# frankenz/Deep-convolutional-neural-network-ResNet-26-and-Attention-network

Measured on AMD Instinct MI355X. Metric: tiles/sec fwd+bwd, 256x256x3 bags, ResNet-26+attn, higher is better.
Workload: dtype bf16; 1 GPU; 8 bags x 256 tiles @256x256x3 per GPU, ResNet-26 (20/40/60/80) + attention-MIL head, fwd+bwd full-bag path (BASELINE.json configs[1]); global_bags=8, tiles_per_bag=256, tile=256, parallelism=bag-parallel dp1, one RCCL all-reduce of the flat 2.56 MB gradient bucket

## Files before the change

deep-convolutional-neural-network-resnet-26-and-attention-network_amd/csrc/conv_resident.hip:

```cpp
#include "pf_common.cuh"
#include <cstdlib>

struct ResConv {
    const __bf16* w;
    const float* bias;
    const __bf16* res;
    const __bf16* act;
    __bf16* out;
    int lrelu;
};
#define MIL_CHAIN_MAX 6
struct ResArgs {
    const __bf16* x;
    ResConv conv[MIL_CHAIN_MAX];
    int nconv;
    int n_img, ngroups;
    unsigned bytes;
    float slope;
};

constexpr int MIL_RES_BDEPTH = 2;

template <int C, int S, int IMGS>
struct ResGeom {
    static constexpr int CG = C / 8, NT = C / 16;
    static constexpr int PIX = mil_pix_pitch(C, 2);
    static constexpr int HS = S + 2;
    static constexpr int IMG = HS * HS * PIX;
    static constexpr int TILE = IMGS * IMG;
    static constexpr int KSTEPS = (9 * CG + 3) / 4;
    static constexpr int NPIX = IMGS * S * S;
    static constexpr int TILES = (NPIX + 15) / 16;
    static constexpr int MW = ((TILES + 7) / 8 + 1) / 2 * 2;
    static constexpr bool RAGGED = (S * S) % 16 != 0 || TILES != 8 * MW;
    static constexpr int NPIECE = NPIX * CG;
    static constexpr int NP = (NPIECE + 511) / 512;
    static constexpr bool WAVE_IS_IMAGE = !RAGGED && (S * S / 16 == MW);
    static_assert(C % 16 == 0, "shape");
    static_assert(TILE <= 160 * 1024, "LDS");
};

template <int C, int S, int IMGS>
__global__ __launch_bounds__(512, 2) void conv_resident_kernel(ResArgs a) {
    using G = ResGeom<C, S, IMGS>;
    constexpr int CG = G::CG, NT = G::NT, PIX = G::PIX, HS = G::HS, IMG = G::IMG, KSTEPS = G::KSTEPS, MW = G::MW, NP = G::NP, NPIX = G::NPIX;
    extern __shared__ __attribute__((aligned(16))) char tile[];
    MIL_POISON(tile);
    const int tid = threadIdx.x, lane = tid & 63;
    const int wave = __builtin_amdgcn_readfirstlane(tid >> 6);
    const int r = lane & 15, gq = lane >> 4;
    const __amdgpu_buffer_rsrc_t rs_x = mil_rsrc(a.x, a.bytes);

    unsigned sink = 0;
    for (int k = 0; k < a.nconv; ++k) {
        const __amdgpu_buffer_rsrc_t rs_wk = mil_rsrc(a.conv[k].w, KSTEPS * NT * 1024);
        for (int line = tid; line < KSTEPS * NT * 8; line += 512)
            sink ^= __builtin_amdgcn_raw_buffer_load_b32(rs_wk, (unsigned)line * 128u, 0, 0);
    }
    {
        constexpr int NB = 4 * S + 4, PPR = PIX / 16;
        for (int idx = tid; idx < IMGS * NB * PPR; idx += 512) {
            const int bp = idx / PPR, j = idx - bp * PPR;
            const int im = bp / NB, b = bp - im * NB;
            int hy, hx;
            if (b < HS) { hy = 0; hx = b; }
            else if (b < 2 * HS) { hy = HS - 1; hx = b - HS; }
            else { hy = 1 + ((b - 2 * HS) >> 1); hx = ((b - 2 * HS) & 1) * (HS - 1); }
            *reinterpret_cast<u32x4_t*>(tile + im * IMG + (hy * HS + hx) * PIX + j * 16) = u32x4_t{0u, 0u, 0u, 0u};
        }
    }
    int pixbase[MW];
#pragma unroll
    for (int m = 0; m < MW; ++m) {
        int P = (wave * MW + m) * 16 + r;
        if (G::RAGGED && P >= NPIX) P = NPIX - 1;
        const int im = P / (S * S), p = P - im * (S * S);
        pixbase[m] = im * IMG + ((p / S) * HS + (p % S)) * PIX;
    }
    const int c_off = (gq >> 1) * 16;

    for (int grp = blockIdx.x; grp < a.ngroups; grp += gridDim.x) {
        const int img0 = grp * IMGS;
        if (grp != (int)blockIdx.x) __syncthreads();
        {
            u32x4_t v[NP];
            const unsigned g0 = (unsigned)img0 * (unsigned)(S * S * C * 2);
#pragma unroll
            for (int i = 0; i < NP; ++i) v[i] = __builtin_amdgcn_raw_buffer_load_b128(rs_x, g0 + (unsigned)(tid + 512 * i) * 16u, 0, 0);
#pragma unroll
            for (int i = 0; i < NP; ++i) {
                const int idx = tid + 512 * i, pl = idx / CG, j = idx - pl * CG;
                const int im = pl / (S * S), p = pl - im * (S * S);
                if (!G::RAGGED || idx < G::NPIECE)
                    *reinterpret_cast<u32x4_t*>(tile + im * IMG + (((p / S) + 1) * HS + (p % S) + 1) * PIX + j * 16) = v[i];
            }
        }

        auto run_conv = [&](const ResConv& cv, bool to_lds, bool first) {
            const __amdgpu_buffer_rsrc_t rs_w = mil_rsrc(cv.w, KSTEPS * NT * 1024);
            const __amdgpu_buffer_rsrc_t rs_res = mil_rsrc(cv.res, cv.res ? a.bytes : 0);
            const __amdgpu_buffer_rsrc_t rs_act = mil_rsrc(cv.act, cv.act ? a.bytes : 0);
            const __amdgpu_buffer_rsrc_t rs_out = mil_rsrc(cv.out, a.bytes);
            f32x4_t acc[MW][NT];
#pragma unroll
            for (int nt = 0; nt < NT; ++nt) {
                f32x4_t b;
#pragma unroll
                for (int i = 0; i < 4; ++i) b[i] = cv.bias ? cv.bias[nt * 16 + gq * 4 + i] : 0.f;
#pragma unroll
                for (int m = 0; m < MW; ++m) acc[m][nt] = b;
            }
            constexpr int BD = MIL_RES_BDEPTH;
            Frag8<BF16> bq[BD + 1][NT], aq[2][MW];
            auto fetch_b = [&](int ks) {
#pragma unroll
                for (int nt = 0; nt < NT; ++nt)
                    bq[ks % (BD + 1)][nt].v = __builtin_bit_cast(bf16x8_t, __builtin_amdgcn_raw_buffer_load_b128(rs_w, (unsigned)(lane * 16), (ks * NT + nt) * 1024, 0));
            };
            auto off_ks = [&](int ks) {
                const int q = 4 * ks + gq;
                const int tap = q / CG, cg = q - tap * CG;
                const int ty = (tap * 11) >> 5, tx = tap - ty * 3;
                return q < 9 * CG ? (ty * HS + tx) * PIX + cg * 16 : 0;
            };
            auto fetch_a = [&](int ks) {
                const int off = off_ks(ks);
#pragma unroll
                for (int m = 0; m < MW; ++m) aq[ks & 1][m] = lds_frag<BF16>(tile + pixbase[m] + off);
            };
#pragma unroll
            for (int ks = 0; ks < BD; ++ks) fetch_b(ks);
            if (first || !G::WAVE_IS_IMAGE) __syncthreads();
            fetch_a(0);
#pragma unroll
            for (int ks = 0; ks < KSTEPS; ++ks) {
                if (ks + BD < KSTEPS) fetch_b(ks + BD);
                if (ks + 1 < KSTEPS) fetch_a(ks + 1);
                __builtin_amdgcn_sched_barrier(0);
#pragma unroll
                for (int m = 0; m < MW; ++m)
#pragma unroll
                    for (int nt = 0; nt < NT; ++nt) acc[m][nt] = mma8(bq[ks % (BD + 1)][nt], aq[ks & 1][m], acc[m][nt]);
                __builtin_amdgcn_sched_barrier(0);
            }
            if (to_lds && !G::WAVE_IS_IMAGE) __syncthreads();
#pragma unroll
            for (int p = 0; p < MW / 2; ++p) {
                const int P = (wave * MW + 2 * p + (gq & 1)) * 16 + r;
                const bool in_list = !G::RAGGED || P < NPIX;
                const int Pc = in_list ? P : NPIX - 1, im = Pc / (S * S), px = Pc - im * (S * S);
                const bool img_ok = in_list && img0 + im < a.n_img;
                const unsigned goff = img_ok ? (unsigned)(((img0 + im) * (S * S) + px) * (C * 2) + c_off) : MIL_OOB;
                u32x4_t rr[NT], ra[NT];
#pragma unroll
                for (int nt = 0; nt < NT; ++nt) {
                    if (cv.res) rr[nt] = __builtin_amdgcn_raw_buffer_load_b128(rs_res, goff == MIL_OOB ? MIL_OOB : goff + nt * 32, 0, 0);
                    if (cv.act) ra[nt] = __builtin_amdgcn_raw_buffer_load_b128(rs_act, goff == MIL_OOB ? MIL_OOB : goff + nt * 32, 0, 0);
                }
                const int loff = im * IMG + (((px / S) + 1) * HS + (px % S) + 1) * PIX + c_off;
#pragma unroll
                for (int nt = 0; nt < NT; ++nt) {
                    float v[8];
#pragma unroll
                    for (int i = 0; i < 4; ++i) {
                        float lo = acc[2 * p][nt][i], hi = acc[2 * p + 1][nt][i];
                        if (i == 0) mil_swap16<true>(lo, hi); else mil_swap16<false>(lo, hi);
                        v[i] = lo;
                        v[4 + i] = hi;
                    }
                    if (cv.res) {
                        const bf16x8_t tt = __builtin_bit_cast(bf16x8_t, rr[nt]);
#pragma unroll
                        for (int i = 0; i < 8; ++i) v[i] += (float)tt[i];
                    }
                    if (cv.lrelu) {
#pragma unroll
                        for (int i = 0; i < 8; ++i) v[i] = fmaxf(v[i], v[i] * a.slope);
                    }
                    if (cv.act) {
                        const bf16x8_t tt = __builtin_bit_cast(bf16x8_t, ra[nt]);
#pragma unroll
                        for (int i = 0; i < 8; ++i) v[i] *= ((float)tt[i] > 0.f ? 1.f : a.slope);
                    }
                    bf16x8_t ov;
#pragma unroll
                    for (int i = 0; i < 8; ++i) ov[i] = (__bf16)v[i];
                    const u32x4_t ou = __builtin_bit_cast(u32x4_t, ov);
                    __builtin_amdgcn_raw_buffer_store_b128(ou, rs_out, goff == MIL_OOB ? MIL_OOB : goff + nt * 32, 0, 0);
                    if (to_lds && in_list) *reinterpret_cast<u32x4_t*>(tile + loff + nt * 32) = img_ok ? ou : u32x4_t{0u, 0u, 0u, 0u};
                }
            }
        };
#pragma unroll 1
        for (int k = 0; k < a.nconv; ++k) run_conv(a.conv[k], k + 1 < a.nconv, k == 0);
    }
    asm volatile("" :: "v"(sink));
}

static int mil_res_grid_cap(int grid) {
    const char* e = mil_test_knob("MIL_RES_GRID_CAP");
    const int cap = e ? atoi(e) : 0;
    return (cap > 0 && grid > cap) ? cap : grid;
}

#include "conv_resident_x3.cuh"

template <int C, int S, int IMGS>
static int launch_resident(ResArgs a, hipStream_t st) {
    using G = ResGeom<C, S, IMGS>;
    auto kern = conv_resident_kernel<C, S, IMGS>;
    if (hipFuncSetAttribute(reinterpret_cast<const void*>(kern), hipFuncAttributeMaxDynamicSharedMemorySize, G::TILE) != hipSuccess)
        return MIL_ERR_LAUNCH;
    a.ngroups = (a.n_img + IMGS - 1) / IMGS;
    int grid = mil_num_cus();
    if (grid > a.ngroups) grid = a.ngroups;
    grid = mil_res_grid_cap(grid);
    hipLaunchKernelGGL(kern, dim3(grid), dim3(512), G::TILE, st, a);
    MIL_CHECK_LAUNCH();
    return MIL_OK;
}

static int resident_dispatch(ResArgs a, int cp, int H, int W, hipStream_t st) {
    if ((size_t)a.n_img * H * W * cp * 2 >= ((size_t)1 << 31)) return MIL_ERR_UNSUPPORTED;
    a.bytes = (unsigned)((size_t)a.n_img * H * W * cp * 2);
    if (cp == 80 && H == 8 && W == 8) return launch_resident<80, 8, 8>(a, st);
    if (cp == 64 && H == 16 && W == 16) return launch_resident<64, 16, 3>(a, st);
    if (cp == 80 && H == 10 && W == 10) return launch_resident<80, 10, 5>(a, st);
    if (cp == 64 && H == 19 && W == 19) return launch_resident<64, 19, 2>(a, st);
    return MIL_ERR_UNSUPPORTED;
}

int mil_resident_conv(const void* x, const void* wpack, const float* bias_pad, const void* res, const void* act, void* y, int n_img,
                      int H, int W, int cp, int apply_lrelu, float slope, hipStream_t st) {
    if (n_img <= 0 || slope < 0.f || slope >= 1.f) return MIL_ERR_UNSUPPORTED;
    if (cp != 80) return MIL_ERR_UNSUPPORTED;
    ResArgs a{};
    a.x = (const __bf16*)x; a.n_img = n_img; a.slope = slope; a.nconv = 1;
    a.conv[0].w = (const __bf16*)wpack; a.conv[0].bias = bias_pad; a.conv[0].res = (const __bf16*)res; a.conv[0].act = (const __bf16*)act;
    a.conv[0].out = (__bf16*)y; a.conv[0].lrelu = apply_lrelu;
    return resident_dispatch(a, cp, H, W, st);
}

int mil_resident_conv_x3(const void* x, const void* wpack, const float* bias_pad, const void* res, const void* act, void* y, int n_img,
                         int H, int W, int cp, int apply_lrelu, float slope, hipStream_t st) {
    if (n_img <= 0 || slope < 0.f || slope >= 1.f) return MIL_ERR_UNSUPPORTED;
    ResArgsX3 a{};
    a.x = (const float*)x; a.n_img = n_img; a.slope = slope; a.nconv = 1;
    a.conv[0].w = (const char*)wpack; a.conv[0].bias = bias_pad; a.conv[0].res = (const float*)res; a.conv[0].act = (const float*)act;
    a.conv[0].out = (float*)y; a.conv[0].lrelu = apply_lrelu;
    return resident_dispatch_x3(a, cp, H, W, st);
}

struct MilChainConv {
    const void* wpack; const float* bias; const void* res; const void* act; void* out; int lrelu; int pad_;
};
extern "C" int mil_conv_chain(const void* x, const MilChainConv* convs, int nconv, int n_img, int H, int W, int cp, float slope,
                              int dtype, void* stream) {
    if (!x || !convs || nconv < 1 || nconv > MIL_CHAIN_MAX || n_img < 0) return MIL_ERR_ARG;
    for (int k = 0; k < nconv; ++k) if (!convs[k].wpack || !convs[k].out) return MIL_ERR_ARG;
    if ((dtype != MIL_DT_BF16 && dtype != MIL_DT_F32S) || slope < 0.f || slope >= 1.f) return MIL_ERR_UNSUPPORTED;
    if (n_img == 0) return MIL_OK;
    if (dtype == MIL_DT_F32S) {
        ResArgsX3 b{};
        b.x = (const float*)x; b.n_img = n_img; b.slope = slope; b.nconv = nconv;
        for (int k = 0; k < nconv; ++k) {
            b.conv[k].w = (const char*)convs[k].wpack; b.conv[k].bias = convs[k].bias; b.conv[k].res = (const float*)convs[k].res;
            b.conv[k].act = (const float*)convs[k].act; b.conv[k].out = (float*)convs[k].out; b.conv[k].lrelu = convs[k].lrelu;
        }
        return resident_dispatch_x3(b, cp, H, W, reinterpret_cast<hipStream_t>(stream));
    }
    ResArgs a{};
    a.x = (const __bf16*)x; a.n_img = n_img; a.slope = slope; a.nconv = nconv;
    for (int k = 0; k < nconv; ++k) {
        a.conv[k].w = (const __bf16*)convs[k].wpack; a.conv[k].bias = convs[k].bias; a.conv[k].res = (const __bf16*)convs[k].res;
        a.conv[k].act = (const __bf16*)convs[k].act; a.conv[k].out = (__bf16*)convs[k].out; a.conv[k].lrelu = convs[k].lrelu;
    }
    return resident_dispatch(a, cp, H, W, reinterpret_cast<hipStream_t>(stream));
}

extern "C" int mil_conv_pair(const void* x, const void* wpackA, const float* biasA, const void* resA, const void* actA,
                             int lreluA, void* outA, const void* wpackB, const float* biasB, const void* resB,
                             const void* actB, int lreluB, void* outB, int n_img, int H, int W, int cp, float slope,
                             int dtype, void* stream) {
    if (!x || !wpackA || !wpackB || !outA || !outB || n_img < 0) return MIL_ERR_ARG;
    const MilChainConv c[2] = {{wpackA, biasA, resA, actA, outA, lreluA, 0}, {wpackB, biasB, resB, actB, outB, lreluB, 0}};
    return mil_conv_chain(x, c, 2, n_img, H, W, cp, slope, dtype, stream);
}
```

deep-convolutional-neural-network-resnet-26-and-attention-network_amd/ops.py:

```python
import ctypes

import torch

from . import _lib as L

LEAK = 0.1


class KernelTimer:

    def __init__(self, want):
        self.want = want
        self.spans = []

    def bracket(self, label):
        if not self.want(label):
            return None
        start = torch.cuda.Event(enable_timing=True)
        end = torch.cuda.Event(enable_timing=True)
        start.record()
        self.spans.append((label, start, end))
        return end

    def durations_ms(self):
        torch.cuda.synchronize()
        return [(label, s.elapsed_time(e)) for label, s, e in self.spans]


TIMER = None


class ReduceBatch:
    MAX_JOBS = 64

    def __init__(self, device):
        self.device = device
        self.rec = L.lib().mil_reduce_job_bytes()
        self.host = (ctypes.c_char * (self.rec * self.MAX_JOBS))()
        self.dev = torch.empty(self.rec * self.MAX_JOBS, dtype=torch.uint8, device=device)
        self.uploaded = None
        self.ws = {}
        self.handed = None

    def workspace(self, key, nbytes):
        if self.handed is not None:
            if key in self.handed:
                raise RuntimeError(f"slab workspace {key!r} handed out twice inside one deferred-reduction block: the second "
                                   "producer would overwrite slabs the batched reduction has not read yet")
            self.handed.add(key)
        t = self.ws.get(key)
        if t is None or t.numel() * 4 < nbytes:
            t = self.ws[key] = torch.empty((nbytes + 3) // 4, dtype=torch.float32, device=self.device)
        return t

    def __enter__(self):
        L.check(L.lib().mil_reduce_defer_begin(ctypes.addressof(self.host), self.MAX_JOBS), "mil_reduce_defer_begin")
        self.handed = set()
        return self

    def __exit__(self, exc_type, exc, tb):
        n = ctypes.c_int(0)
        self.handed = None
        L.check(L.lib().mil_reduce_defer_end(ctypes.byref(n)), "mil_reduce_defer_end")
        if exc_type is not None or n.value == 0:
            return False
        raw = bytes(self.host[: self.rec * n.value])
        if raw != self.uploaded:
            self.dev[: len(raw)].copy_(torch.frombuffer(bytearray(raw), dtype=torch.uint8))
            self.uploaded = raw
        L.check(L.lib().mil_wgrad_reduce_all(self.dev.data_ptr(), ctypes.addressof(self.host), n.value, L.stream_ptr()),
                "mil_wgrad_reduce_all")
        return False


def cpad(c):
    return (c + 7) // 8 * 8


def _need(t, shape, dtype, name):
    if t is None:
        return
    if not t.is_cuda or not t.is_contiguous():
        raise ValueError(f"{name} must be a contiguous CUDA tensor")
    if tuple(t.shape) != tuple(shape) or t.dtype != dtype:
        raise ValueError(f"{name}: expected {tuple(shape)} {dtype}, got {tuple(t.shape)} {t.dtype}")


def stem_s2d(x, dtype):
    if x.dim() != 4 or x.shape[1] != 3 or x.dtype != torch.float32 or not x.is_cuda:
        raise ValueError(f"expected a CUDA fp32 [N,3,H,W] tile stack, got {tuple(x.shape)} {x.dtype} on {x.device}")
    x = x.contiguous()
    n, _, h, w = x.shape
    out = torch.empty((n, (h + 1) // 2, (w + 1) // 2, 16), dtype=dtype, device=x.device)
    L.check(L.lib().mil_stem_s2d(x.data_ptr(), out.data_ptr(), n, h, w, L.dt_code(dtype), L.stream_ptr()), "mil_stem_s2d")
    return out


def _need_u8_tiles(x):
    if x.dim() != 4 or x.shape[1] != 3 or x.dtype != torch.uint8 or not x.is_cuda or not x.is_contiguous():
        raise ValueError(f"expected a contiguous CUDA uint8 [N,3,H,W] tile stack, got {tuple(x.shape)} {x.dtype} on {x.device}")


def stem_s2d_u8(x, dtype):
    _need_u8_tiles(x)
    n, _, h, w = x.shape
    out = torch.empty((n, (h + 1) // 2, (w + 1) // 2, 16), dtype=dtype, device=x.device)
    L.check(L.lib().mil_stem_s2d_u8(x.data_ptr(), out.data_ptr(), n, h, w, L.dt_code(dtype), L.stream_ptr()), "mil_stem_s2d_u8")
    return out


def pack_weights(w, bias, mode, dtype):
    w = w.detach()
    if w.dtype != torch.float32 or not w.is_cuda or w.dim() != 4:
        raise ValueError("weights must be CUDA fp32 [Cout,Cin,k,k]")
    w = w.contiguous()
    cout, cin, ks, _ = w.shape
    elems = ctypes.c_size_t(0)
    L.check(L.lib().mil_packed_weight_elems(ctypes.byref(elems), cout, cin, ks, mode), "mil_packed_weight_elems")
    if dtype == L.BF16X3:
        with L.f32_mma(L.MIL_DT_F32S):
            return pack_weights(w, bias, mode, torch.float32)
    packed = torch.empty(elems.value, dtype=dtype, device=w.device)
    n_out = cin if mode == L.PACK_DGRAD else cout
    nt = (cpad(n_out) + 15) // 16
    bias_pad = torch.empty(nt * 16, dtype=torch.float32, device=w.device)
    b = None if bias is None else bias.detach().contiguous()
    L.check(L.lib().mil_pack_conv_weights(w.data_ptr(), L.ptr(b), packed.data_ptr(), bias_pad.data_ptr(), cout, cin, ks,
                                          mode, L.dt_code(dtype, mma=True), L.stream_ptr()), "mil_pack_conv_weights")
    return packed, bias_pad


def conv(x, wpack, bias_pad, cout_p, *, ks, stride, pad, out_hw=None, res=None, act=None, lrelu=False,
         zero_insert=False, slope=LEAK):
    n, h, w, cin_p = x.shape
    if zero_insert:
        if out_hw is None:
            raise ValueError("zero_insert needs the full-resolution output size")
        ho, wo = out_hw
    else:
        ho = (h + 2 * pad - ks) // stride + 1 if ks != 4 else h
        wo = (w + 2 * pad - ks) // stride + 1 if ks != 4 else w
    y = torch.empty((n, ho, wo, cout_p), dtype=x.dtype, device=x.device)
    _need(x, x.shape, x.dtype, "x")
    _need(res, y.shape, x.dtype, "res")
    _need(act, y.shape, x.dtype, "act")
    end = TIMER.bracket(("conv", cin_p, cout_p, ks, stride, bool(zero_insert), n, ho, wo)) if TIMER else None
    L.check(L.lib().mil_conv_igemm(x.data_ptr(), wpack.data_ptr(), L.ptr(bias_pad), L.ptr(res), L.ptr(act), y.data_ptr(),
                                   n, h, w, cin_p, ho, wo, cout_p, ks, 1 if zero_insert else stride, pad,
                                   1 if zero_insert else 0, 1 if lrelu else 0, slope, L.dt_code(x.dtype, mma=True), L.stream_ptr()),
            "mil_conv_igemm")
    if end is not None:
        end.record()
    return y


def wgrad_workspace_bytes(n, h, w, cin, ho, wo, cout, ks, stride, pad, stem, dtype):
    need = ctypes.c_size_t(0)
    L.check(L.lib().mil_conv_wgrad_workspace(ctypes.byref(need), n, h, w, cin, ho, wo, cout, ks, stride, pad,
                                             1 if stem else 0, L.dt_code(dtype, mma=True)), "mil_conv_wgrad_workspace")
    return need.value


def conv_wgrad(x, dz, cin, cout, *, ks, stride, pad, stem=False, want_bias=True, workspace=None, out=None):
    n, h, w, cin_p = x.shape
    _, ho, wo, cout_p = dz.shape
    _need(dz, (n, ho, wo, cpad(cout)), x.dtype, "dz")
    _need(x, (n, h, w, 16 if stem else cpad(cin)), x.dtype, "x")
    need = wgrad_workspace_bytes(n, h, w, cin, ho, wo, cout, ks, stride, pad, stem, x.dtype)
    if workspace is None or workspace.numel() * workspace.element_size() < need:
        workspace = torch.empty((need + 3) // 4, dtype=torch.float32, device=x.device)
    kk = 7 if stem else ks
    if out is None:
        dw = torch.empty((cout, cin, kk, kk), dtype=torch.float32, device=x.device)
        db = torch.empty(cout, dtype=torch.float32, device=x.device) if want_bias else None
    else:
        dw, db = out
        _need(dw, (cout, cin, kk, kk), torch.float32, "dw")
        _need(db, (cout,), torch.float32, "db")
    end = TIMER.bracket(("wgrad", cin_p, cout_p, ks, stride, n, ho, wo)) if TIMER else None
    L.check(L.lib().mil_conv_wgrad(x.data_ptr(), dz.data_ptr(), dw.data_ptr(), L.ptr(db), workspace.data_ptr(),
                                   workspace.numel() * workspace.element_size(), n, h, w, cin, ho, wo, cout, ks, stride,
                                   pad, 1 if stem else 0, 0 if out is None else 1, L.dt_code(x.dtype, mma=True), L.stream_ptr()),
            "mil_conv_wgrad")
    if end is not None:
        end.record()
    return dw, db


def bwd_fused_workspace_bytes(n, h, w, cout, cin, ks, pad, dtype, dense=False):
    need = ctypes.c_size_t(0)
    rc = L.lib().mil_conv_bwd_fused_workspace(ctypes.byref(need), n, h, w, cout, cin, ks, pad, L.dt_code(dtype, dense, mma=True))
    if rc == 2:
        return None
    L.check(rc, "mil_conv_bwd_fused_workspace")
    return need.value


def conv_bwd_fused(dz, wpack_dgrad, x, cin, cout, *, addend=None, mask=True, ks=3, pad=1, workspace=None, slope=LEAK,
                   out=None):
    n, h, w, cz = dz.shape
    dense = cz == cout and cpad(cout) != cout
    need = bwd_fused_workspace_bytes(n, h, w, cout, cin, ks, pad, dz.dtype, dense)
    if need is None:
        return None
    _need(dz, (n, h, w, cout if dense else cpad(cout)), dz.dtype, "dz")
    _need(x, (n, h, w, cpad(cin)), dz.dtype, "x")
    _need(addend, (n, h, w, cin if dense else cpad(cin)), dz.dtype, "addend")
    if workspace is None or workspace.numel() * workspace.element_size() < need:
        workspace = torch.empty((need + 3) // 4, dtype=torch.float32, device=dz.device)
    dx = torch.empty((n, h, w, cin), dtype=dz.dtype, device=dz.device) if dense else torch.empty_like(x)
    if out is None:
        dw = torch.empty((cout, cin, ks, ks), dtype=torch.float32, device=dz.device)
        db = torch.empty(cout, dtype=torch.float32, device=dz.device)
    else:
        dw, db = out
        _need(dw, (cout, cin, ks, ks), torch.float32, "dw")
        _need(db, (cout,), torch.float32, "db")
    end = TIMER.bracket(("bwd_fused", cpad(cout), cpad(cin), ks, 1, False, n, h, w, addend is not None)) if TIMER else None
    L.check(L.lib().mil_conv_bwd_fused(dz.data_ptr(), wpack_dgrad.data_ptr(), x.data_ptr(), L.ptr(addend), dx.data_ptr(),
                                       dw.data_ptr(), db.data_ptr(), workspace.data_ptr(),
                                       workspace.numel() * workspace.element_size(), n, h, w, cout, cin, ks, pad,
                                       1 if mask else 0, 0 if out is None else 1, slope, L.dt_code(dz.dtype, dense, mma=True), L.stream_ptr()),
            "mil_conv_bwd_fused")
    if end is not None:
        end.record()
    return dx, dw, db


def maxpool_fwd(x):
    n, h, w, cp = x.shape
    ho, wo = (h - 1) // 2 + 1, (w - 1) // 2 + 1
    y = torch.empty((n, ho, wo, cp), dtype=x.dtype, device=x.device)
    widx = torch.empty((n, ho, wo, cp), dtype=torch.uint8, device=x.device)
    L.check(L.lib().mil_maxpool_fwd(x.data_ptr(), y.data_ptr(), widx.data_ptr(), n, h, w, cp, L.dt_code(x.dtype),
                                    L.stream_ptr()), "mil_maxpool_fwd")
    return y, widx


def maxpool_bwd(gy, widx, in_hw, lrelu_mask=True, slope=LEAK):
    n, ho, wo, cp = widx.shape
    h, w = in_hw
    if ((h - 1) // 2 + 1, (w - 1) // 2 + 1) != (ho, wo):
        raise ValueError(f"pool input {h}x{w} does not produce {ho}x{wo}")
    _need(gy, widx.shape, gy.dtype, "gy")
    gx = torch.empty((n, h, w, cp), dtype=gy.dtype, device=gy.device)
    L.check(L.lib().mil_maxpool_bwd(gy.data_ptr(), widx.data_ptr(), gx.data_ptr(), n, h, w, cp, 1 if lrelu_mask else 0,
                                    slope, L.dt_code(gy.dtype), L.stream_ptr()), "mil_maxpool_bwd")
    return gx


BLOCK_FWD_CHANNELS = (24,)


def conv_block_fwd(x, wpack1, bias1, wpack2, bias2, *, slope=LEAK):
    n, h, w, cp = x.shape
    code = L.dt_code(x.dtype, mma=True)
    if code == L.MIL_DT_F32S:
        if cp != 24 or h < 8 or w < 16:
            return None
    elif x.dtype != torch.bfloat16 or cp not in BLOCK_FWD_CHANNELS or h < 16 or w < 16:
        return None
    _need(x, x.shape, x.dtype, "x")
    o1 = torch.empty_like(x)
    y = torch.empty_like(x)
    end = TIMER.bracket(("block_fwd", cp, n, h, w)) if TIMER else None
    rc = L.lib().mil_conv_block_fwd(x.data_ptr(), wpack1.data_ptr(), L.ptr(bias1), wpack2.data_ptr(), L.ptr(bias2),
                                    o1.data_ptr(), y.data_ptr(), n, h, w, cp, slope, code, L.stream_ptr())
    if rc == 2:
        return None
    L.check(rc, "mil_conv_block_fwd")
    if end is not None:
        end.record()
    return o1, y


RESIDENT_SHAPES = ((80, 8, 8), (64, 16, 16), (80, 10, 10), (64, 19, 19))


class _ChainConv(ctypes.Structure):
    _fields_ = [("wpack", ctypes.c_void_p), ("bias", ctypes.c_void_p), ("res", ctypes.c_void_p), ("act", ctypes.c_void_p),
                ("out", ctypes.c_void_p), ("lrelu", ctypes.c_int), ("pad_", ctypes.c_int)]


def conv_chain(x, convs, *, slope=LEAK):
    n, h, w, cp = x.shape
    code = L.dt_code(x.dtype, mma=True)
    if code not in (L.MIL_DT_BF16, L.MIL_DT_F32S) or (cp, h, w) not in RESIDENT_SHAPES or not 1 <= len(convs) <= 6:
        return None
    _need(x, x.shape, x.dtype, "x")
    outs = [torch.empty_like(x) for _ in convs]
    arr = (_ChainConv * len(convs))()
    for k, c in enumerate(convs):
        ops_ = {}
        for name in ("res", "act"):
            t = c.get(name)
            if isinstance(t, int):
                if not 0 <= t < k:
                    raise ValueError(f"conv {k}: {name} refers to conv {t}, which is not earlier in the chain")
                t = outs[t]
            _need(t, x.shape, x.dtype, name)
            ops_[name] = t
        arr[k].wpack = c["w"].data_ptr()
        arr[k].bias = L.ptr(c.get("bias"))
        arr[k].res, arr[k].act = L.ptr(ops_["res"]), L.ptr(ops_["act"])
        arr[k].out = outs[k].data_ptr()
        arr[k].lrelu = 1 if c.get("lrelu") else 0
    end = TIMER.bracket(("chain", cp, n, h, w, len(convs))) if TIMER else None
    rc = L.lib().mil_conv_chain(x.data_ptr(), ctypes.addressof(arr), len(convs), n, h, w, cp, slope, code, L.stream_ptr())
    if rc == 2:
        return None
    L.check(rc, "mil_conv_chain")
    if end is not None:
        end.record()
    return outs


def conv_pair(x, wA, biasA, wB, biasB, *, resA=None, actA=None, lreluA=False, resB=None, actB=None, lreluB=False, slope=LEAK):
    outs = conv_chain(x, [dict(w=wA, bias=biasA, res=resA, act=actA, lrelu=lreluA),
                          dict(w=wB, bias=biasB, res=resB, act=actB, lrelu=lreluB)], slope=slope)
    return None if outs is None else (outs[0], outs[1])


def conv_s2_entry(x, wpack3, bias_pad, wpack1, cout_p, *, slope=LEAK):
    n, h, w, cin_p = x.shape
    code = L.dt_code(x.dtype, mma=True)
    if code not in (L.MIL_DT_BF16, L.MIL_DT_F32S):
        return None
    _need(x, x.shape, x.dtype, "x")
    ho, wo = (h - 1) // 2 + 1, (w - 1) // 2 + 1
    y1 = torch.empty((n, ho, wo, cout_p), dtype=x.dtype, device=x.device)
    y2 = torch.empty_like(y1)
    end = TIMER.bracket(("s2_entry", cin_p, cout_p, n, h, w)) if TIMER else None
    rc = L.lib().mil_conv_s2_entry(x.data_ptr(), wpack3.data_ptr(), L.ptr(bias_pad), wpack1.data_ptr(), y1.data_ptr(),
                                   y2.data_ptr(), n, h, w, cin_p, cout_p, slope, code, L.stream_ptr())
    if rc == 2:
        return None
    L.check(rc, "mil_conv_s2_entry")
    if end is not None:
        end.record()
    return y1, y2


def conv_wgrad_pair(x, dz1, dz2, cin, cout, *, workspace=None, out=None):
    n, h, w, _ = x.shape
    _, ho, wo, _ = dz1.shape
    code = L.dt_code(x.dtype, mma=True)
    if code not in (L.MIL_DT_BF16, L.MIL_DT_F32S):
        return None
    _need(x, (n, h, w, cpad(cin)), x.dtype, "x")
    _need(dz1, (n, ho, wo, cpad(cout)), x.dtype, "dz1")
    _need(dz2, (n, ho, wo, cpad(cout)), x.dtype, "dz2")
    need = ctypes.c_size_t(0)
    rc = L.lib().mil_conv_wgrad_pair_workspace(ctypes.byref(need), n, h, w, cin, ho, wo, cout, code)
    if rc == 2:
        return None
    L.check(rc, "mil_conv_wgrad_pair_workspace")
    if workspace is None or workspace.numel() * workspace.element_size() < need.value:
        workspace = torch.empty((need.value + 3) // 4, dtype=torch.float32, device=x.device)
    if out is None:
        dw3 = torch.empty((cout, cin, 3, 3), dtype=torch.float32, device=x.device)
        db3 = torch.empty(cout, dtype=torch.float32, device=x.device)
        dw1 = torch.empty((cout, cin, 1, 1), dtype=torch.float32, device=x.device)
    else:
        dw3, db3, dw1 = out
        _need(dw3, (cout, cin, 3, 3), torch.float32, "dw3")
        _need(db3, (cout,), torch.float32, "db3")
        _need(dw1, (cout, cin, 1, 1), torch.float32, "dw1")
    rc = L.lib().mil_conv_wgrad_pair(x.data_ptr(), dz1.data_ptr(), dz2.data_ptr(), dw3.data_ptr(), db3.data_ptr(), dw1.data_ptr(),
                                     workspace.data_ptr(), workspace.numel() * workspace.element_size(), n, h, w, cin, ho, wo,
                                     cout, 0 if out is None else 1, code, L.stream_ptr())
    if rc == 2:
        return None
    L.check(rc, "mil_conv_wgrad_pair")
    return dw3, db3, dw1, workspace


def conv_dgrad_s2(dz1, dz2, wpack, cx_p, out_hw, *, act=None, slope=LEAK, dense_cx=None):
    n, h, w, cz_p = dz1.shape
    hh, ww = out_hw
    dense = dense_cx is not None
    if dz1.dtype != torch.bfloat16 and L.dt_code(dz1.dtype, mma=True) != L.MIL_DT_F32S:
        return None
    _need(dz1, dz1.shape, dz1.dtype, "dz1")
    _need(dz2, dz1.shape, dz1.dtype, "dz2")
    y = torch.empty((n, hh, ww, dense_cx if dense else cx_p), dtype=dz1.dtype, device=dz1.device)
    _need(act, (n, hh, ww, cx_p), dz1.dtype, "act")
    end = TIMER.bracket(("dgrad_s2", cz_p, cx_p, n, hh, ww)) if TIMER else None
    rc = L.lib().mil_conv_dgrad_s2(dz1.data_ptr(), L.ptr(dz2), wpack.data_ptr(), L.ptr(act), y.data_ptr(), n, h, w, cz_p,
                                   hh, ww, cx_p, slope, L.dt_code(dz1.dtype, dense, mma=True), L.stream_ptr())
    if rc == 2:
        return None
    L.check(rc, "mil_conv_dgrad_s2")
    if end is not None:
        end.record()
    return y


def stem_fwd_fused(x, wpack, bias_pad, cout_p, *, slope=LEAK, dtype=torch.bfloat16, keep_s2d=True):
    if x.dim() != 4 or x.shape[1] != 3 or x.dtype != torch.float32 or not x.is_cuda:
        raise ValueError(f"expected a CUDA fp32 [N,3,H,W] tile stack, got {tuple(x.shape)} {x.dtype} on {x.device}")
    x = x.contiguous()
    n, c, h, w = x.shape
    code = L.dt_code(dtype, mma=True)
    if code == L.MIL_DT_F32S:
        if keep_s2d or cout_p != 24:
            return None
    elif dtype != torch.bfloat16:
        return None
    if h % 2 or w % 4 or cout_p not in (24, 64) or x.data_ptr() % 16:
        return None
    h2, w2 = h // 2, w // 2
    hp, wp = (h2 - 1) // 2 + 1, (w2 - 1) // 2 + 1
    xs = torch.empty((n, h2, w2, 16), dtype=dtype, device=x.device) if keep_s2d else None
    pool = torch.empty((n, hp, wp, cout_p), dtype=dtype, device=x.device)
    widx = torch.empty((n, hp, wp, cout_p), dtype=torch.uint8, device=x.device)
    end = TIMER.bracket(("stem_fwd", cout_p, n, h, w)) if TIMER else None
    rc = L.lib().mil_stem_fwd_fused(x.data_ptr(), wpack.data_ptr(), L.ptr(bias_pad), L.ptr(xs), pool.data_ptr(),
                                    widx.data_ptr(), n, h, w, cout_p, slope, code, L.stream_ptr())
    if rc == 2:
        return None
    L.check(rc, "mil_stem_fwd_fused")
    if end is not None:
        end.record()
    return xs, pool, widx


def stem_fwd_fused_u8(x, wpack, bias_pad, cout_p, *, slope=LEAK, dtype=torch.bfloat16):
    _need_u8_tiles(x)
    n, c, h, w = x.shape
    code = L.dt_code(dtype, mma=True)
    if code == L.MIL_DT_F32S:
        if cout_p != 24:
            return None
    elif dtype != torch.bfloat16:
        return None
    if h % 2 or w % 4 or cout_p not in (24, 64) or x.data_ptr() % 4:
        return None
    h2, w2 = h // 2, w // 2
    hp, wp = (h2 - 1) // 2 + 1, (w2 - 1) // 2 + 1
    pool = torch.empty((n, hp, wp, cout_p), dtype=dtype, device=x.device)
    widx = torch.empty((n, hp, wp, cout_p), dtype=torch.uint8, device=x.device)
    end = TIMER.bracket(("stem_fwd_u8", cout_p, n, h, w)) if TIMER else None
    rc = L.lib().mil_stem_fwd_fused_u8(x.data_ptr(), wpack.data_ptr(), L.ptr(bias_pad), pool.data_ptr(), widx.data_ptr(), n, h, w,
                                       cout_p, slope, code, L.stream_ptr())
    if rc == 2:
        return None
    L.check(rc, "mil_stem_fwd_fused_u8")
    if end is not None:
        end.record()
    return pool, widx


def stem_fwd_fused_xs(xs, wpack, bias_pad, cout_p, *, slope=LEAK):
    if xs.dim() != 4 or xs.shape[3] != 16 or xs.dtype != torch.bfloat16 or not xs.is_cuda or not xs.is_contiguous():
        raise ValueError(f"expected a contiguous CUDA bf16 [N,H/2,W/2,16] tensor, got {tuple(xs.shape)} {xs.dtype}")
    n, h2, w2, _ = xs.shape
    if cout_p not in (24, 64) or xs.data_ptr() % 16:
        return None
    hp, wp = (h2 - 1) // 2 + 1, (w2 - 1) // 2 + 1
    pool = torch.empty((n, hp, wp, cout_p), dtype=torch.bfloat16, device=xs.device)
    widx = torch.empty((n, hp, wp, cout_p), dtype=torch.uint8, device=xs.device)
    end = TIMER.bracket(("stem_fwd_xs", cout_p, n, 2 * h2, 2 * w2)) if TIMER else None
    rc = L.lib().mil_stem_fwd_fused_xs(xs.data_ptr(), wpack.data_ptr(), L.ptr(bias_pad), pool.data_ptr(), widx.data_ptr(), n, h2, w2,
                                       cout_p, slope, L.MIL_DT_BF16, L.stream_ptr())
    if rc == 2:
        return None
    L.check(rc, "mil_stem_fwd_fused_xs")
    if end is not None:
        end.record()
    return pool, widx


def stem_bwd_fused(xs, g_pool, widx, *, workspace=None, out=None, slope=LEAK, ws_alloc=None):
    n, h2, w2, c = xs.shape
    dense = g_pool.shape[-1] == 20
    need = ctypes.c_size_t(0)
    rc = L.lib().mil_stem_bwd_fused_workspace(ctypes.byref(need), n, h2, w2, L.dt_code(xs.dtype, dense))
    if rc == 2:
        return None
    L.check(rc, "mil_stem_bwd_fused_workspace")
    hp, wp = (h2 - 1) // 2 + 1, (w2 - 1) // 2 + 1
    _need(xs, (n, h2, w2, 16), xs.dtype, "xs")
    _need(g_pool, (n, hp, wp, 20 if dense else 24), xs.dtype, "g_pool")
    _need(widx, (n, hp, wp, 24), torch.uint8, "widx")
    if ws_alloc is not None:
        workspace = ws_alloc(need.value)
    if workspace is None or workspace.numel() * workspace.element_size() < need.value:
        workspace = torch.empty((need.value + 3) // 4, dtype=torch.float32, device=xs.device)
    if out is None:
        dw = torch.empty((20, 3, 7, 7), dtype=torch.float32, device=xs.device)
        db = torch.empty(20, dtype=torch.float32, device=xs.device)
    else:
        dw, db = out
        _need(dw, (20, 3, 7, 7), torch.float32, "dw")
        _need(db, (20,), torch.float32, "db")
    end = TIMER.bracket(("stem_bwd_xs", n, 2 * h2, 2 * w2)) if TIMER else None
    L.check(L.lib().mil_stem_bwd_fused(xs.data_ptr(), g_pool.data_ptr(), widx.data_ptr(), dw.data_ptr(), db.data_ptr(),
                                       workspace.data_ptr(), workspace.numel() * workspace.element_size(), n, h2, w2,
                                       slope, 0 if out is None else 1, L.dt_code(xs.dtype, dense), L.stream_ptr()),
            "mil_stem_bwd_fused")
    if end is not None:
        end.record()
    return dw, db


def stem_bwd_fused_nchw(x, g_pool, widx, *, workspace=None, out=None, slope=LEAK, ws_alloc=None):
    if x.dim() != 4 or x.shape[1] != 3 or x.dtype != torch.float32 or not x.is_cuda or not x.is_contiguous():
        return None
    n, _, h, w = x.shape
    dense = g_pool.shape[-1] == 20
    need = ctypes.c_size_t(0)
    rc = L.lib().mil_stem_bwd_fused_nchw_workspace(ctypes.byref(need), n, h, w, L.dt_code(g_pool.dtype, dense, mma=True))
    if rc == 2 or x.data_ptr() % 16:
        return None
    L.check(rc, "mil_stem_bwd_fused_nchw_workspace")
    h2, w2 = h // 2, w // 2
    hp, wp = (h2 - 1) // 2 + 1, (w2 - 1) // 2 + 1
    _need(g_pool, (n, hp, wp, 20 if dense else 24), g_pool.dtype, "g_pool")
    _need(widx, (n, hp, wp, 24), torch.uint8, "widx")
    if ws_alloc is not None:
        workspace = ws_alloc(need.value)
    if workspace is None or workspace.numel() * workspace.element_size() < need.value:
        workspace = torch.empty((need.value + 3) // 4, dtype=torch.float32, device=x.device)
    if out is None:
        dw = torch.empty((20, 3, 7, 7), dtype=torch.float32, device=x.device)
        db = torch.empty(20, dtype=torch.float32, device=x.device)
    else:
        dw, db = out
        _need(dw, (20, 3, 7, 7), torch.float32, "dw")
        _need(db, (20,), torch.float32, "db")
    end = TIMER.bracket(("stem_bwd", n, h, w)) if TIMER else None
    rc = L.lib().mil_stem_bwd_fused_nchw(x.data_ptr(), g_pool.data_ptr(), widx.data_ptr(), dw.data_ptr(), db.data_ptr(),
                                         workspace.data_ptr(), workspace.numel() * workspace.element_size(), n, h, w,
                                         slope, 0 if out is None else 1, L.dt_code(g_pool.dtype, dense, mma=True), L.stream_ptr())
    if rc == 2:
        return None
    L.check(rc, "mil_stem_bwd_fused_nchw")
    if end is not None:
        end.record()
    return dw, db


def stem_bwd_fused_u8(x, g_pool, widx, *, workspace=None, out=None, slope=LEAK, ws_alloc=None):
    if x.dim() != 4 or x.shape[1] != 3 or x.dtype != torch.uint8 or not x.is_cuda or not x.is_contiguous():
        return None
    n, _, h, w = x.shape
    dense = g_pool.shape[-1] == 20
    need = ctypes.c_size_t(0)
    rc = L.lib().mil_stem_bwd_fused_u8_workspace(ctypes.byref(need), n, h, w, L.dt_code(g_pool.dtype, dense, mma=True))
    if rc == 2 or x.data_ptr() % 4:
        return None
    L.check(rc, "mil_stem_bwd_fused_u8_workspace")
    h2, w2 = h // 2, w // 2
    hp, wp = (h2 - 1) // 2 + 1, (w2 - 1) // 2 + 1
    _need(g_pool, (n, hp, wp, 20 if dense else 24), g_pool.dtype, "g_pool")
    _need(widx, (n, hp, wp, 24), torch.uint8, "widx")
    if ws_alloc is not None:
        workspace = ws_alloc(need.value)
    if workspace is None or workspace.numel() * workspace.element_size() < need.value:
        workspace = torch.empty((need.value + 3) // 4, dtype=torch.float32, device=x.device)
    if out is None:
        dw = torch.empty((20, 3, 7, 7), dtype=torch.float32, device=x.device)
        db = torch.empty(20, dtype=torch.float32, device=x.device)
    else:
        dw, db = out
        _need(dw, (20, 3, 7, 7), torch.float32, "dw")
        _need(db, (20,), torch.float32, "db")
    end = TIMER.bracket(("stem_bwd_u8", n, h, w)) if TIMER else None
    rc = L.lib().mil_stem_bwd_fused_u8(x.data_ptr(), g_pool.data_ptr(), widx.data_ptr(), dw.data_ptr(), db.data_ptr(),
                                       workspace.data_ptr(), workspace.numel() * workspace.element_size(), n, h, w,
                                       slope, 0 if out is None else 1, L.dt_code(g_pool.dtype, dense, mma=True), L.stream_ptr())
    if rc == 2:
        return None
    L.check(rc, "mil_stem_bwd_fused_u8")
    if end is not None:
        end.record()
    return dw, db


def stem_bwd_dense_ok(src, dtype):
    need = ctypes.c_size_t(0)
    if src.dim() == 4 and src.shape[1] == 3 and src.dtype == torch.uint8:
        n, _, h, w = src.shape
        if not src.is_contiguous() or src.data_ptr() % 4:
            return False
        return L.lib().mil_stem_bwd_fused_u8_workspace(ctypes.byref(need), n, h, w, L.dt_code(dtype, True, mma=True)) == 0
    if src.dim() == 4 and src.shape[1] == 3 and src.dtype == torch.float32:
        n, _, h, w = src.shape
        if not src.is_contiguous() or src.data_ptr() % 16:
            return False
        return L.lib().mil_stem_bwd_fused_nchw_workspace(ctypes.byref(need), n, h, w, L.dt_code(dtype, True, mma=True)) == 0
    n, h2, w2, _ = src.shape
    if dtype != torch.bfloat16:
# ... 115 lines not shown
```

Measured before the change: 256,400 tiles/s.

## Balance resident conv work per block and prefetch epilogue operands early

Replaces the strided group loop with a contiguous, evenly divided run of images per block, so partial trailing groups only process the pixels they actually have. Waves with no work skip the MMA loop and epilogue, and per-pair tiles beyond the live count are skipped. Residual and activation operands are prefetched during the last k-steps and double-buffered, and the epilogue is specialised at compile time on whether res/act exist. The risks are extra register pressure from the double-buffered operand registers and more complex dynamic control flow. ops.py also gains an optional preallocated outs argument.

```diff
diff --git a/deep-convolutional-neural-network-resnet-26-and-attention-network_amd/csrc/conv_resident.hip b/deep-convolutional-neural-network-resnet-26-and-attention-network_amd/csrc/conv_resident.hip
--- a/deep-convolutional-neural-network-resnet-26-and-attention-network_amd/csrc/conv_resident.hip
+++ b/deep-convolutional-neural-network-resnet-26-and-attention-network_amd/csrc/conv_resident.hip
@@ -1,5 +1,6 @@
 #include "pf_common.cuh"
 #include <cstdlib>
+#include <type_traits>
 
 struct ResConv {
     const __bf16* w;
@@ -14,7 +15,7 @@
     const __bf16* x;
     ResConv conv[MIL_CHAIN_MAX];
     int nconv;
-    int n_img, ngroups;
+    int n_img;
     unsigned bytes;
     float slope;
 };
@@ -43,7 +44,7 @@
 template <int C, int S, int IMGS>
 __global__ __launch_bounds__(512, 2) void conv_resident_kernel(ResArgs a) {
     using G = ResGeom<C, S, IMGS>;
-    constexpr int CG = G::CG, NT = G::NT, PIX = G::PIX, HS = G::HS, IMG = G::IMG, KSTEPS = G::KSTEPS, MW = G::MW, NP = G::NP, NPIX = G::NPIX;
+    constexpr int CG = G::CG, NT = G::NT, PIX = G::PIX, HS = G::HS, IMG = G::IMG, KSTEPS = G::KSTEPS, MW = G::MW, NP = G::NP;
     extern __shared__ __attribute__((aligned(16))) char tile[];
     MIL_POISON(tile);
     const int tid = threadIdx.x, lane = tid & 63;
@@ -69,31 +70,55 @@
             *reinterpret_cast<u32x4_t*>(tile + im * IMG + (hy * HS + hx) * PIX + j * 16) = u32x4_t{0u, 0u, 0u, 0u};
         }
     }
-    int pixbase[MW];
-#pragma unroll
-    for (int m = 0; m < MW; ++m) {
-        int P = (wave * MW + m) * 16 + r;
-        if (G::RAGGED && P >= NPIX) P = NPIX - 1;
-        const int im = P / (S * S), p = P - im * (S * S);
-        pixbase[m] = im * IMG + ((p / S) * HS + (p % S)) * PIX;
-    }
     const int c_off = (gq >> 1) * 16;
 
-    for (int grp = blockIdx.x; grp < a.ngroups; grp += gridDim.x) {
-        const int img0 = grp * IMGS;
-        if (grp != (int)blockIdx.x) __syncthreads();
-        {
-            u32x4_t v[NP];
-            const unsigned g0 = (unsigned)img0 * (unsigned)(S * S * C * 2);
-#pragma unroll
-            for (int i = 0; i < NP; ++i) v[i] = __builtin_amdgcn_raw_buffer_load_b128(rs_x, g0 + (unsigned)(tid + 512 * i) * 16u, 0, 0);
-#pragma unroll
-            for (int i = 0; i < NP; ++i) {
-                const int idx = tid + 512 * i, pl = idx / CG, j = idx - pl * CG;
-                const int im = pl / (S * S), p = pl - im * (S * S);
-                if (!G::RAGGED || idx < G::NPIECE)
-                    *reinterpret_cast<u32x4_t*>(tile + im * IMG + (((p / S) + 1) * HS + (p % S) + 1) * PIX + j * 16) = v[i];
-            }
+    const int per = a.n_img / (int)gridDim.x, extra = a.n_img - per * (int)gridDim.x;
+    const int run0 = (int)blockIdx.x * per + ((int)blockIdx.x < extra ? (int)blockIdx.x : extra);
+    const int run_n = per + ((int)blockIdx.x < extra ? 1 : 0);
+
+    u32x4_t v[NP];
+    auto fetch_group = [&](int img0, int gi) {
+        const unsigned g0 = (unsigned)img0 * (unsigned)(S * S * C * 2);
+        const int npiece = gi * (S * S * CG);
+        int tid_g = tid;
+        asm volatile("" : "+v"(tid_g));
+#pragma unroll
+        for (int i = 0; i < NP; ++i) {
+            const int idx = tid_g + 512 * i;
+            v[i] = __builtin_amdgcn_raw_buffer_load_b128(rs_x, idx < npiece ? g0 + (unsigned)idx * 16u : MIL_OOB, 0, 0);
+        }
+    };
+    asm volatile("" :: "v"(sink));
+
+    for (int done = 0; done < run_n; done += IMGS) {
+        const int img0 = run0 + done;
+        const int gi = run_n - done < IMGS ? run_n - done : IMGS;
+        const int npix_g = gi * (S * S);
+        const int tiles_g = (npix_g + 15) >> 4;
+        const int stride = G::WAVE_IS_IMAGE ? MW : (((tiles_g + 7) >> 3) + 1) & ~1;
+        int mw_live = tiles_g - wave * stride;
+        mw_live = mw_live < 0 ? 0 : (mw_live > stride ? stride : (mw_live + 1) & ~1);
+        const bool live = mw_live > 0;
+        int pixbase[MW];
+        int r_g = r;
+        asm volatile("" : "+v"(r_g));
+#pragma unroll
+        for (int m = 0; m < MW; ++m) {
+            int P = (wave * stride + m) * 16 + r_g;
+            if (P >= npix_g) P = npix_g - 1;
+            const int im = P / (S * S), p = P - im * (S * S);
+            pixbase[m] = im * IMG + ((p / S) * HS + (p % S)) * PIX;
+        }
+        if (done) __syncthreads();
+        fetch_group(img0, gi);
+        int tid_g = tid;
+        asm volatile("" : "+v"(tid_g));
+#pragma unroll
+        for (int i = 0; i < NP; ++i) {
+            const int idx = tid_g + 512 * i, pl = idx / CG, j = idx - pl * CG;
+            const int im = pl / (S * S), p = pl - im * (S * S);
+            if (idx < gi * (S * S * CG))
+                *reinterpret_cast<u32x4_t*>(tile + im * IMG + (((p / S) + 1) * HS + (p % S) + 1) * PIX + j * 16) = v[i];
         }
 
         auto run_conv = [&](const ResConv& cv, bool to_lds, bool first) {
@@ -101,17 +126,12 @@
             const __amdgpu_buffer_rsrc_t rs_res = mil_rsrc(cv.res, cv.res ? a.bytes : 0);
             const __amdgpu_buffer_rsrc_t rs_act = mil_rsrc(cv.act, cv.act ? a.bytes : 0);
             const __amdgpu_buffer_rsrc_t rs_out = mil_rsrc(cv.out, a.bytes);
+            constexpr int BD = MIL_RES_BDEPTH;
+            constexpr bool EARLY_OPS = !G::WAVE_IS_IMAGE;
+            static_assert(KSTEPS > BD, "the epilogue operands are fetched BD k-steps before the end");
             f32x4_t acc[MW][NT];
-#pragma unroll
-            for (int nt = 0; nt < NT; ++nt) {
-                f32x4_t b;
-#pragma unroll
-                for (int i = 0; i < 4; ++i) b[i] = cv.bias ? cv.bias[nt * 16 + gq * 4 + i] : 0.f;
-#pragma unroll
-                for (int m = 0; m < MW; ++m) acc[m][nt] = b;
-            }
-            constexpr int BD = MIL_RES_BDEPTH;
             Frag8<BF16> bq[BD + 1][NT], aq[2][MW];
+            u32x4_t rr[2][NT], ra[2][NT];
             auto fetch_b = [&](int ks) {
 #pragma unroll
                 for (int nt = 0; nt < NT; ++nt)
@@ -126,75 +146,117 @@
             auto fetch_a = [&](int ks) {
                 const int off = off_ks(ks);
 #pragma unroll
-                for (int m = 0; m < MW; ++m) aq[ks & 1][m] = lds_frag<BF16>(tile + pixbase[m] + off);
-            };
-#pragma unroll
-            for (int ks = 0; ks < BD; ++ks) fetch_b(ks);
+                for (int p = 0; p < MW / 2; ++p)
+                    if (p == 0 || 2 * p < mw_live) {
+                        aq[ks & 1][2 * p] = lds_frag<BF16>(tile + pixbase[2 * p] + off);
+                        aq[ks & 1][2 * p + 1] = lds_frag<BF16>(tile + pixbase[2 * p + 1] + off);
+                    }
+            };
+            auto pair_addr = [&](int p, unsigned& goff, int& loff) {
+                int r_p = r;
+                asm volatile("" : "+v"(r_p));
+                const int P = (wave * stride + 2 * p + (gq & 1)) * 16 + r_p;
+                const bool in_list = P < npix_g;
+                const int Pc = in_list ? P : npix_g - 1, im = Pc / (S * S), px = Pc - im * (S * S);
+                goff = in_list ? (unsigned)(((img0 + im) * (S * S) + px) * (C * 2) + c_off) : MIL_OOB;
+                loff = im * IMG + (((px / S) + 1) * HS + (px % S) + 1) * PIX + c_off;
+            };
+            auto fetch_ops = [&](int p, bool want_res, bool want_act) {
+                unsigned goff; int loff;
+                pair_addr(p, goff, loff);
+#pragma unroll
+                for (int nt = 0; nt < NT; ++nt) {
+                    if (want_res) rr[p & 1][nt] = __builtin_amdgcn_raw_buffer_load_b128(rs_res, goff == MIL_OOB ? MIL_OOB : goff + nt * 32, 0, 0);
+                    if (want_act) ra[p & 1][nt] = __builtin_amdgcn_raw_buffer_load_b128(rs_act, goff == MIL_OOB ? MIL_OOB : goff + nt * 32, 0, 0);
+                }
+            };
+            if (live) {
+#pragma unroll
+                for (int nt = 0; nt < NT; ++nt) {
+                    f32x4_t b;
+#pragma unroll
+                    for (int i = 0; i < 4; ++i) b[i] = cv.bias ? cv.bias[nt * 16 + gq * 4 + i] : 0.f;
+#pragma unroll
+                    for (int m = 0; m < MW; ++m) acc[m][nt] = b;
+                }
+#pragma unroll
+                for (int ks = 0; ks < BD; ++ks) fetch_b(ks);
+            }
             if (first || !G::WAVE_IS_IMAGE) __syncthreads();
-            fetch_a(0);
-#pragma unroll
-            for (int ks = 0; ks < KSTEPS; ++ks) {
-                if (ks + BD < KSTEPS) fetch_b(ks + BD);
-                if (ks + 1 < KSTEPS) fetch_a(ks + 1);
-                __builtin_amdgcn_sched_barrier(0);
-#pragma unroll
-                for (int m = 0; m < MW; ++m)
-#pragma unroll
-                    for (int nt = 0; nt < NT; ++nt) acc[m][nt] = mma8(bq[ks % (BD + 1)][nt], aq[ks & 1][m], acc[m][nt]);
-                __builtin_amdgcn_sched_barrier(0);
+            if (live) {
+                fetch_a(0);
+#pragma unroll
+                for (int ks = 0; ks < KSTEPS; ++ks) {
+                    if (ks + BD < KSTEPS) fetch_b(ks + BD);
+                    if (EARLY_OPS && ks + BD == KSTEPS) fetch_ops(0, true, false);
+                    if (EARLY_OPS && ks + 1 == KSTEPS) fetch_ops(0, false, true);
+                    if (ks + 1 < KSTEPS) fetch_a(ks + 1);
+                    __builtin_amdgcn_sched_barrier(0);
+#pragma unroll
+                    for (int p = 0; p < MW / 2; ++p)
+                        if (p == 0 || 2 * p < mw_live) {
+#pragma unroll
+                            for (int m = 2 * p; m < 2 * p + 2; ++m)
+#pragma unroll
+                                for (int nt = 0; nt < NT; ++nt) acc[m][nt] = mma8(bq[ks % (BD + 1)][nt], aq[ks & 1][m], acc[m][nt]);
+                        }
+                    __builtin_amdgcn_sched_barrier(0);
+                }
             }
             if (to_lds && !G::WAVE_IS_IMAGE) __syncthreads();
-#pragma unroll
-            for (int p = 0; p < MW / 2; ++p) {
-                const int P = (wave * MW + 2 * p + (gq & 1)) * 16 + r;
-                const bool in_list = !G::RAGGED || P < NPIX;
-                const int Pc = in_list ? P : NPIX - 1, im = Pc / (S * S), px = Pc - im * (S * S);
-                const bool img_ok = in_list && img0 + im < a.n_img;
-                const unsigned goff = img_ok ? (unsigned)(((img0 + im) * (S * S) + px) * (C * 2) + c_off) : MIL_OOB;
-                u32x4_t rr[NT], ra[NT];
-#pragma unroll
-                for (int nt = 0; nt < NT; ++nt) {
-                    if (cv.res) rr[nt] = __builtin_amdgcn_raw_buffer_load_b128(rs_res, goff == MIL_OOB ? MIL_OOB : goff + nt * 32, 0, 0);
-                    if (cv.act) ra[nt] = __builtin_amdgcn_raw_buffer_load_b128(rs_act, goff == MIL_OOB ? MIL_OOB : goff + nt * 32, 0, 0);
+            auto epilogue = [&](auto has_res, auto has_act) {
+                constexpr bool HAS_RES = decltype(has_res)::value, HAS_ACT = decltype(has_act)::value;
+#pragma unroll
+                for (int p = 0; p < MW / 2; ++p) {
+                    if (p == 0 || 2 * p < mw_live) {
+                        if (!EARLY_OPS) fetch_ops(p, HAS_RES, HAS_ACT);
+                        else if (p + 1 < MW / 2 && 2 * (p + 1) < mw_live) fetch_ops(p + 1, HAS_RES, HAS_ACT);
+                        unsigned goff; int loff;
+                        pair_addr(p, goff, loff);
+#pragma unroll
+                        for (int nt = 0; nt < NT; ++nt) {
+                            float v[8];
+#pragma unroll
+                            for (int i = 0; i < 4; ++i) {
+                                float lo = acc[2 * p][nt][i], hi = acc[2 * p + 1][nt][i];
+                                if (i == 0) mil_swap16<true>(lo, hi); else mil_swap16<false>(lo, hi);
+                                v[i] = lo;
+                                v[4 + i] = hi;
+                            }
+                            if (HAS_RES) {
+                                const bf16x8_t tt = __builtin_bit_cast(bf16x8_t, rr[p & 1][nt]);
+#pragma unroll
+                                for (int i = 0; i < 8; ++i) v[i] += (float)tt[i];
+                            }
+                            if (cv.lrelu) {
+#pragma unroll
+                                for (int i = 0; i < 8; ++i) v[i] = fmaxf(v[i], v[i] * a.slope);
+                            }
+                            if (HAS_ACT) {
+                                const bf16x8_t tt = __builtin_bit_cast(bf16x8_t, ra[p & 1][nt]);
+#pragma unroll
+                                for (int i = 0; i < 8; ++i) v[i] *= ((float)tt[i] > 0.f ? 1.f : a.slope);
+                            }
+                            bf16x8_t ov;
+#pragma unroll
+                            for (int i = 0; i < 8; ++i) ov[i] = (__bf16)v[i];
+                            const u32x4_t ou = __builtin_bit_cast(u32x4_t, ov);
+                            __builtin_amdgcn_raw_buffer_store_b128(ou, rs_out, goff == MIL_OOB ? MIL_OOB : goff + nt * 32, 0, 0);
+                            if (to_lds && goff != MIL_OOB) *reinterpret_cast<u32x4_t*>(tile + loff + nt * 32) = ou;
+                        }
+                    }
                 }
-                const int loff = im * IMG + (((px / S) + 1) * HS + (px % S) + 1) * PIX + c_off;
-#pragma unroll
-                for (int nt = 0; nt < NT; ++nt) {
-                    float v[8];
-#pragma unroll
-                    for (int i = 0; i < 4; ++i) {
-                        float lo = acc[2 * p][nt][i], hi = acc[2 * p + 1][nt][i];
-                        if (i == 0) mil_swap16<true>(lo, hi); else mil_swap16<false>(lo, hi);
-                        v[i] = lo;
-                        v[4 + i] = hi;
-                    }
-                    if (cv.res) {
-                        const bf16x8_t tt = __builtin_bit_cast(bf16x8_t, rr[nt]);
-#pragma unroll
-                        for (int i = 0; i < 8; ++i) v[i] += (float)tt[i];
-                    }
-                    if (cv.lrelu) {
-#pragma unroll
-                        for (int i = 0; i < 8; ++i) v[i] = fmaxf(v[i], v[i] * a.slope);
-                    }
-                    if (cv.act) {
-                        const bf16x8_t tt = __builtin_bit_cast(bf16x8_t, ra[nt]);
-#pragma unroll
-                        for (int i = 0; i < 8; ++i) v[i] *= ((float)tt[i] > 0.f ? 1.f : a.slope);
-                    }
-                    bf16x8_t ov;
-#pragma unroll
-                    for (int i = 0; i < 8; ++i) ov[i] = (__bf16)v[i];
-                    const u32x4_t ou = __builtin_bit_cast(u32x4_t, ov);
-                    __builtin_amdgcn_raw_buffer_store_b128(ou, rs_out, goff == MIL_OOB ? MIL_OOB : goff + nt * 32, 0, 0);
-                    if (to_lds && in_list) *reinterpret_cast<u32x4_t*>(tile + loff + nt * 32) = img_ok ? ou : u32x4_t{0u, 0u, 0u, 0u};
-                }
+            };
+            if (live) {
+                using T = std::true_type;
+                using F = std::false_type;
+                if (cv.res) { if (cv.act) epilogue(T{}, T{}); else epilogue(T{}, F{}); }
+                else { if (cv.act) epilogue(F{}, T{}); else epilogue(F{}, F{}); }
             }
         };
 #pragma unroll 1
         for (int k = 0; k < a.nconv; ++k) run_conv(a.conv[k], k + 1 < a.nconv, k == 0);
     }
-    asm volatile("" :: "v"(sink));
 }
 
 static int mil_res_grid_cap(int grid) {
@@ -211,9 +273,9 @@
     auto kern = conv_resident_kernel<C, S, IMGS>;
     if (hipFuncSetAttribute(reinterpret_cast<const void*>(kern), hipFuncAttributeMaxDynamicSharedMemorySize, G::TILE) != hipSuccess)
         return MIL_ERR_LAUNCH;
-    a.ngroups = (a.n_img + IMGS - 1) / IMGS;
+    const int ngroups = (a.n_img + IMGS - 1) / IMGS;
     int grid = mil_num_cus();
-    if (grid > a.ngroups) grid = a.ngroups;
+    if (grid > ngroups) grid = ngroups;
     grid = mil_res_grid_cap(grid);
     hipLaunchKernelGGL(kern, dim3(grid), dim3(512), G::TILE, st, a);
     MIL_CHECK_LAUNCH();
diff --git a/deep-convolutional-neural-network-resnet-26-and-attention-network_amd/ops.py b/deep-convolutional-neural-network-resnet-26-and-attention-network_amd/ops.py
--- a/deep-convolutional-neural-network-resnet-26-and-attention-network_amd/ops.py
+++ b/deep-convolutional-neural-network-resnet-26-and-attention-network_amd/ops.py
@@ -282,13 +282,18 @@
                 ("out", ctypes.c_void_p), ("lrelu", ctypes.c_int), ("pad_", ctypes.c_int)]
 
 
-def conv_chain(x, convs, *, slope=LEAK):
+def conv_chain(x, convs, *, slope=LEAK, outs=None):
     n, h, w, cp = x.shape
     code = L.dt_code(x.dtype, mma=True)
     if code not in (L.MIL_DT_BF16, L.MIL_DT_F32S) or (cp, h, w) not in RESIDENT_SHAPES or not 1 <= len(convs) <= 6:
         return None
     _need(x, x.shape, x.dtype, "x")
-    outs = [torch.empty_like(x) for _ in convs]
+    if outs is None:
+        outs = [torch.empty_like(x) for _ in convs]
+    elif len(outs) != len(convs):
+        raise ValueError(f"{len(outs)} outputs for {len(convs)} convs")
+    for k, o in enumerate(outs):
+        _need(o, x.shape, x.dtype, f"outs[{k}]")
     arr = (_ChainConv * len(convs))()
     for k, c in enumerate(convs):
         ops_ = {}
```

Measured after the change: 257,400 tiles/s, median of 6. About the same (+0.4%).
